# XiSHEN0220/RANSAC-Flow

Hardware: AMD Instinct MI355X
Metric: aligned image-pairs/sec @480×640, 1/2/4/8 MI355X; max-abs flow Δ vs ref (higher is better)
Workload: dtype f32

## Files before the change

### ransac-flow_amd/csrc/conv1x1s.hip

```cpp
#include "common.h"
#include "conv_epilogue.h"
#include "conv_split.h"
#include "conv_tile.h"
#include "group.h"

namespace {

struct C1SArgs {
    const float* in; const u32x4* wS; const float* scale; const float* shift; const float* res; float* out;
    int Cin, HW, Cout, act, Mpad;
    long long P;
    int tilesM, tilesP;
    int stride, Win, Wo, HWin;
};

template <int TM, int WM>
__device__ __forceinline__ void conv1x1_split_body(const C1SArgs& a, const unsigned bx, const unsigned) {
    constexpr int BM = 32 * TM * WM, BN = 128, KB = 16, NT = 128 * WM;
    constexpr bool WIDE = WM == 4;
    __shared__ u32x4 As[2][3][2][BM];
    __shared__ u32x4 Bs[2][3][2][BN];
    __shared__ float s_scale[BM], s_shift[BM];

    const int t = threadIdx.x, lane = t & 63, wave = t >> 6;
    const int wm = wave >> 1, wn = wave & 1;
    const int lrow = lane >> 5, lcol = lane & 31;
    const size_t HW = (size_t)a.HW, HWin = (size_t)a.HWin;
    const int nk = a.Cin / KB;

    const int bid = xcd_remap(bx, a.tilesM * a.tilesP);
    const int m0 = (bid % a.tilesM) * BM;
    const long long n0 = (long long)(bid / a.tilesM) * BN;
    SplitWeights<BM, NT> wa;
    wa.init(a.wS, a.Mpad, m0, WIDE);
    constexpr int NB = 2048 / NT;
    const int bh = t >> 7, bp = t & 127;
    const float* bsrc;
    {
        long long p = n0 + bp;
        if (p >= a.P) p = a.P - 1;
        const long long n = p / a.HW;
        int off = (int)(p - n * a.HW);
        if (a.stride != 1) { const int y = off / a.Wo, x = off - y * a.Wo; off = y * a.stride * a.Win + x * a.stride; }
        bsrc = a.in + ((size_t)n * a.Cin + NB * bh) * HWin + (size_t)off;
    }
    float rb[NB];
    auto load_stage = [&](int kb) {
        wa.load(kb, a.Mpad);
#pragma unroll
        for (int i = 0; i < NB; ++i) rb[i] = bsrc[(size_t)(kb * KB + i) * HWin];
    };
    auto store_stage = [&](int buf) {
        wa.store(&As[buf][0][0][0]);
        if constexpr (NB == 8) {
            u32x4 hi, mid, lo;
            split_word(rb, hi, mid, lo);
            Bs[buf][0][bh][bp] = hi;
            Bs[buf][1][bh][bp] = mid;
            Bs[buf][2][bh][bp] = lo;
        } else {
            u32x2 hi, mid, lo;
            split_word(rb, hi, mid, lo);
            u32x2* w = reinterpret_cast<u32x2*>(&Bs[buf][0][bh >> 1][bp]) + (bh & 1);
            w[0] = hi;
            w[4 * BN] = mid;
            w[8 * BN] = lo;
        }
    };
    stage_bn<BM>(s_scale, s_shift, a.scale, a.shift, m0, a.Cout);
    load_stage(0);
    store_stage(0);
    if (nk > 1) load_stage(1);
    __syncthreads();

    f32x16 acc[TM][2], low[TM][2];
    acc_zero(acc);
    acc_zero(low);

    for (int s = 0; s < nk; ++s) {
        const int cur = s & 1;
        bf16x8 af[3][TM], bf[3][2];
#pragma unroll
        for (int pc = 0; pc < 3; ++pc) {
#pragma unroll
            for (int i = 0; i < TM; ++i) af[pc][i] = as_frag(As[cur][pc][lrow][wm * TM * 32 + i * 32 + lcol]);
#pragma unroll
            for (int j = 0; j < 2; ++j) bf[pc][j] = as_frag(Bs[cur][pc][lrow][wn * 64 + j * 32 + lcol]);
        }
        if (s + 1 < nk) store_stage(cur ^ 1);
        if (s + 2 < nk) load_stage(s + 2);
        __builtin_amdgcn_sched_barrier(0);
#pragma unroll
        for (int i = 0; i < TM; ++i)
#pragma unroll
            for (int j = 0; j < 2; ++j) {
                low[i][j] = __builtin_amdgcn_mfma_f32_32x32x16_bf16(af[2][i], bf[0][j], low[i][j], 0, 0, 0);
                low[i][j] = __builtin_amdgcn_mfma_f32_32x32x16_bf16(af[0][i], bf[2][j], low[i][j], 0, 0, 0);
                low[i][j] = __builtin_amdgcn_mfma_f32_32x32x16_bf16(af[1][i], bf[1][j], low[i][j], 0, 0, 0);
            }
#pragma unroll
        for (int i = 0; i < TM; ++i)
#pragma unroll
            for (int j = 0; j < 2; ++j) {
                low[i][j] = __builtin_amdgcn_mfma_f32_32x32x16_bf16(af[1][i], bf[0][j], low[i][j], 0, 0, 0);
                low[i][j] = __builtin_amdgcn_mfma_f32_32x32x16_bf16(af[0][i], bf[1][j], low[i][j], 0, 0, 0);
                acc[i][j] = __builtin_amdgcn_mfma_f32_32x32x16_bf16(af[0][i], bf[0][j], acc[i][j], 0, 0, 0);
            }
        __builtin_amdgcn_sched_barrier(0);
        __syncthreads();
    }
    acc_add(acc, low);

    size_t pix_off[2];
    bool pix_ok[2];
    pix_linear<2>(pix_off, pix_ok, n0 + wn * 64 + lcol, a.P, a.HW, a.Cout);
    conv_epilogue<TM, 2, false>(acc, s_scale, s_shift, a.res, a.out, a.act, a.Cout, HW, m0, wm, lrow, pix_off, pix_ok, m0 + BM <= a.Cout);
}

template <int TM> using Split1 = RfxFamily<C1SArgs, conv1x1_split_body<TM, 2>, 256, 2>;
using Split1Wide = RfxFamily<C1SArgs, conv1x1_split_body<2, 4>, 512, 1>;

template <int TM>
__global__ __launch_bounds__((Split1<TM>::BLOCK), (Split1<TM>::min_waves())) void conv1x1_split_kernel(C1SArgs a) {
    conv1x1_split_body<TM, 2>(a, blockIdx.x, gridDim.x);
}

__global__ __launch_bounds__(Split1Wide::BLOCK, Split1Wide::min_waves()) void conv1x1_split_wide_kernel(C1SArgs a) {
    conv1x1_split_body<2, 4>(a, blockIdx.x, gridDim.x);
}

int c1s_tile_channels(long long P, int Cin, int Cout) {
    static const int mode = [] { const char* e = getenv("RFX_C1S_WIDE"); return e ? (atoi(e) == 0 ? 0 : 1) : -1; }();
    static const long long cus = [] {
        int dev = 0, n = 256;
        if (hipGetDevice(&dev) == hipSuccess) hipDeviceGetAttribute(&n, hipDeviceAttributeMultiprocessorCount, dev);
        return (long long)(n > 0 ? n : 256);
    }();
    if (Cout <= 64) return 64;
    if (Cout < 256 || mode == 0) return 128;
    if (mode == 1) return 256;
    if (Cin < 512) return 128;
    const long long tp = (P + 127) / 128, w = (Cout + 255) / 256 * tp, n = (Cout + 127) / 128 * tp;
    const long long rest = n % (2 * cus);
    const long long cost_wide = (w + cus - 1) / cus * 81, cost_128 = n / (2 * cus) * 100 + (rest == 0 ? 0 : rest <= cus ? 58 : 100);
    return cost_wide < cost_128 ? 256 : 128;
}

template <int TM, int WM>
int launch_split(C1SArgs& a, hipStream_t st) {
    constexpr int BM = 32 * TM * WM;
    a.tilesM = (a.Cout + BM - 1) / BM;
    a.tilesP = (int)((a.P + 127) / 128);
    const long long nwg = (long long)a.tilesM * a.tilesP;
    if (nwg > 0x7fffffffLL) return RFX_E_LIMIT;
    if constexpr (WM == 4) return Split1Wide::launch(conv1x1_split_wide_kernel, a, (unsigned)nwg, st);
    else return Split1<TM>::launch(conv1x1_split_kernel<TM>, a, (unsigned)nwg, st);
}

}

static int conv1x1_split_launch(const float* in, const void* wS, const float* scale, const float* shift, const float* residual,
                                float* out, int N, int Cin, int Hin, int Win, int Cout, int stride, int act, void* stream) {
    if (const int rc = conv_check_common(in, wS, out, N, Cin, Hin, Win, Cout, act)) return rc;
    if (stride != 1 && stride != 2) return RFX_E_ARG;
    const int Ho = (Hin - 1) / stride + 1, Wo = (Win - 1) / stride + 1;
    C1SArgs a;
    a.in = in; a.wS = reinterpret_cast<const u32x4*>(wS); a.scale = scale; a.shift = shift; a.res = residual; a.out = out;
    a.Cin = Cin; a.HW = Ho * Wo; a.Cout = Cout; a.act = act; a.Mpad = (Cout + 127) / 128 * 128;
    a.P = (long long)N * a.HW;
    a.stride = stride; a.Win = Win; a.Wo = Wo; a.HWin = Hin * Win;
    switch (c1s_tile_channels(a.P, Cin, Cout)) {
        case 256: return launch_split<2, 4>(a, rfx_stream(stream));
        case 128: return launch_split<2, 2>(a, rfx_stream(stream));
        default: return launch_split<1, 2>(a, rfx_stream(stream));
    }
}

extern "C" int rfx_conv1x1_split_tile_channels(int N, int Cin, int HWout, int Cout) {
    if (N <= 0 || Cin <= 0 || HWout <= 0 || Cout <= 0) return RFX_E_ARG;
    return c1s_tile_channels((long long)N * HWout, Cin, Cout);
}

extern "C" int rfx_conv1x1_split_f32(const float* in, const void* wS, const float* scale, const float* shift, const float* residual,
                                     float* out, int N, int Cin, int HW, int Cout, int act, void* stream) {
    return conv1x1_split_launch(in, wS, scale, shift, residual, out, N, Cin, 1, HW, Cout, 1, act, stream);
}

extern "C" int rfx_conv1x1_split_strided_f32(const float* in, const void* wS, const float* scale, const float* shift, const float* residual,
                                             float* out, int N, int Cin, int Hin, int Win, int Cout, int stride, int act, void* stream) {
    return conv1x1_split_launch(in, wS, scale, shift, residual, out, N, Cin, Hin, Win, Cout, stride, act, stream);
}
```

### ransac-flow_amd/csrc/conv_epilogue.h

```cpp
#pragma once
#include "common.h"

template <int TM, int TN>
__device__ __forceinline__ void conv_residual_prefetch(float (&pre)[TM * TN][16], const float* __restrict__ resp, size_t HWo,
                                                       int m0, int wm, int lrow, const size_t (&pix_off)[TN]) {
#pragma unroll
    for (int s = 0; s < TM * TN; ++s) {
        const size_t base = pix_off[s % TN] + (size_t)(m0 + (wm * TM + s / TN) * 32 + 4 * lrow) * HWo;
#pragma unroll
        for (int r = 0; r < 16; ++r) pre[s][r] = resp[base + (size_t)((r & 3) + 8 * (r >> 2)) * HWo];
    }
}

template <int TM, int TN, bool LEAN = false, bool PRE = false>
__device__ __forceinline__ void conv_epilogue(const f32x16 (&acc)[TM][TN], const float* s_scale, const float* s_shift,
                                              const float* __restrict__ resp, float* __restrict__ outp, int act,
                                              int Cout, size_t HWo, int m0, int wm, int lrow,
                                              const size_t (&pix_off)[TN], const bool (&pix_ok)[TN], bool m_full,
                                              const float (*pre)[16] = nullptr) {
    const bool has_res = resp != nullptr;
    if (m_full && act != RFX_ACT_SIGMOID) {
        const bool relu = act == RFX_ACT_RELU;
        constexpr int NS = TM * TN;
        auto sub_base = [&](int s) { return pix_off[s % TN] + (size_t)(m0 + (wm * TM + s / TN) * 32 + 4 * lrow) * HWo; };
        float rv[2][16];
        if (has_res && !LEAN && !PRE) {
            const size_t b0 = sub_base(0);
#pragma unroll
            for (int r = 0; r < 16; ++r) rv[0][r] = resp[b0 + (size_t)((r & 3) + 8 * (r >> 2)) * HWo];
        }
        float sc[16], sh[16];
#pragma unroll
        for (int s = 0; s < NS; ++s) {
            const int i = s / TN, j = s % TN;
            if (j == 0 || LEAN) {
                const int ml0 = (wm * TM + i) * 32 + 4 * lrow;
#pragma unroll
                for (int r = 0; r < 16; ++r) {
                    sc[r] = s_scale[ml0 + (r & 3) + 8 * (r >> 2)];
                    sh[r] = s_shift[ml0 + (r & 3) + 8 * (r >> 2)];
                }
            }
            if (has_res && LEAN && !PRE) {
                const size_t bc = sub_base(s);
#pragma unroll
                for (int r = 0; r < 16; ++r) rv[s & 1][r] = resp[bc + (size_t)((r & 3) + 8 * (r >> 2)) * HWo];
            }
            if (has_res && !LEAN && !PRE && s + 1 < NS) {
                const size_t bn = sub_base(s + 1);
#pragma unroll
                for (int r = 0; r < 16; ++r) rv[(s + 1) & 1][r] = resp[bn + (size_t)((r & 3) + 8 * (r >> 2)) * HWo];
            }
            const size_t base = sub_base(s);
            float v[16];
#pragma unroll
            for (int r = 0; r < 16; ++r) v[r] = fmaf(acc[i][j][r], sc[r], sh[r]);
            if (has_res) {
#pragma unroll
                for (int r = 0; r < 16; ++r) v[r] += PRE ? pre[s][r] : rv[s & 1][r];
            }
            if (relu) {
#pragma unroll
                for (int r = 0; r < 16; ++r) v[r] = v[r] > 0.0f ? v[r] : 0.0f;
            }
            if (pix_ok[j]) {
#pragma unroll
                for (int r = 0; r < 16; ++r) outp[base + (size_t)((r & 3) + 8 * (r >> 2)) * HWo] = v[r];
            }
            __builtin_amdgcn_sched_barrier(0);
        }
        return;
    }
#pragma unroll
    for (int j = 0; j < TN; ++j) {
#pragma unroll
        for (int i = 0; i < TM; ++i) {
            float rv[16];
#pragma unroll
            for (int r = 0; r < 16; ++r) {
                const int ml = (wm * TM + i) * 32 + (r & 3) + 8 * (r >> 2) + 4 * lrow;
                const int mc = (m0 + ml < Cout) ? (m0 + ml) : (Cout - 1);
                rv[r] = has_res ? resp[pix_off[j] + (size_t)mc * HWo] : 0.0f;
            }
#pragma unroll
            for (int r = 0; r < 16; ++r) {
                const int ml = (wm * TM + i) * 32 + (r & 3) + 8 * (r >> 2) + 4 * lrow;
                const int m = m0 + ml;
                float v = fmaf(acc[i][j][r], s_scale[ml], s_shift[ml]);
                if (has_res) v += rv[r];
                if (act == RFX_ACT_RELU) v = v > 0.0f ? v : 0.0f;
                else if (act == RFX_ACT_SIGMOID) v = 1.0f / (1.0f + expf(-v));
                if (pix_ok[j] && m < Cout) outp[pix_off[j] + (size_t)m * HWo] = v;
            }
        }
    }
}
```

### ransac-flow_amd/csrc/conv_tile.h

```cpp
#pragma once
#include "common.h"

template <int BM>
static __device__ __forceinline__ void stage_bn(float* s_scale, float* s_shift, const float* scale, const float* shift, int m0, int Cout) {
    const int t = threadIdx.x;
    if (t < BM) {
        const int m = m0 + t;
        s_scale[t] = (scale && m < Cout) ? scale[m] : 1.0f;
        s_shift[t] = (shift && m < Cout) ? shift[m] : 0.0f;
    }
}

template <int TM, int TN>
static __device__ __forceinline__ void acc_zero(f32x16 (&acc)[TM][TN]) {
#pragma unroll
    for (int i = 0; i < TM; ++i)
#pragma unroll
        for (int j = 0; j < TN; ++j)
#pragma unroll
            for (int r = 0; r < 16; ++r) acc[i][j][r] = 0.0f;
}
template <int TM, int TN>
static __device__ __forceinline__ void acc_add(f32x16 (&acc)[TM][TN], const f32x16 (&low)[TM][TN]) {
#pragma unroll
    for (int i = 0; i < TM; ++i)
#pragma unroll
        for (int j = 0; j < TN; ++j)
#pragma unroll
            for (int r = 0; r < 16; ++r) acc[i][j][r] += low[i][j][r];
}
template <int TM, int TN>
static __device__ __forceinline__ void acc_close_chunk(f32x16 (&tot)[TM][TN], f32x16 (&acc)[TM][TN]) {
#pragma unroll
    for (int i = 0; i < TM; ++i)
#pragma unroll
        for (int j = 0; j < TN; ++j)
#pragma unroll
            for (int r = 0; r < 16; ++r) { tot[i][j][r] += acc[i][j][r]; acc[i][j][r] = 0.0f; }
}

template <int TN>
static __device__ __forceinline__ void pix_linear(size_t (&pix_off)[TN], bool (&pix_ok)[TN], long long p0, long long P, int HW, int Cout) {
#pragma unroll
    for (int j = 0; j < TN; ++j) {
        long long pp = p0 + j * 32;
        pix_ok[j] = pp < P;
        if (!pix_ok[j]) pp = P - 1;
        const long long n = pp / HW;
        pix_off[j] = (size_t)n * Cout * (size_t)HW + (size_t)(pp - n * HW);
    }
}
```

Baseline: 165.6.

## Switch 1x1 split conv to 16x16x32 MFMA with triple-buffered two-step K loop

Replaces the 32x32x16 bf16 MFMA tiles with 16x16x32 ones, reorganising fragments so each iteration consumes two K blocks (one per lane group) from a triple-buffered shared-memory ring. Odd K counts are padded with a zero stage. Global loads and LDS stores are interleaved inside the row loop to overlap with MFMA work, and a new epilogue handles the 4-element accumulator layout. The aim is better MFMA throughput and latency hiding, at the cost of more shared memory (3 buffers) and more accumulator registers, which may reduce occupancy.

```diff
diff --git a/ransac-flow_amd/csrc/conv1x1s.hip b/ransac-flow_amd/csrc/conv1x1s.hip
--- a/ransac-flow_amd/csrc/conv1x1s.hip
+++ b/ransac-flow_amd/csrc/conv1x1s.hip
@@ -16,17 +16,17 @@
 
 template <int TM, int WM>
 __device__ __forceinline__ void conv1x1_split_body(const C1SArgs& a, const unsigned bx, const unsigned) {
-    constexpr int BM = 32 * TM * WM, BN = 128, KB = 16, NT = 128 * WM;
+    constexpr int BM = 32 * TM * WM, BN = 128, KB = 16, NT = 128 * WM, MI = 2 * TM, NJ = 4;
     constexpr bool WIDE = WM == 4;
-    __shared__ u32x4 As[2][3][2][BM];
-    __shared__ u32x4 Bs[2][3][2][BN];
+        __shared__ u32x4 As[3][3][2][BM];
+    __shared__ u32x4 Bs[3][3][2][BN];
     __shared__ float s_scale[BM], s_shift[BM];
 
     const int t = threadIdx.x, lane = t & 63, wave = t >> 6;
     const int wm = wave >> 1, wn = wave & 1;
-    const int lrow = lane >> 5, lcol = lane & 31;
+    const int g = lane >> 4, r16 = lane & 15;
     const size_t HW = (size_t)a.HW, HWin = (size_t)a.HWin;
-    const int nk = a.Cin / KB;
+    const int nk = a.Cin / KB, nkp = (nk + 1) & ~1;
 
     const int bid = xcd_remap(bx, a.tilesM * a.tilesP);
     const int m0 = (bid % a.tilesM) * BM;
@@ -46,9 +46,15 @@
     }
     float rb[NB];
     auto load_stage = [&](int kb) {
-        wa.load(kb, a.Mpad);
-#pragma unroll
-        for (int i = 0; i < NB; ++i) rb[i] = bsrc[(size_t)(kb * KB + i) * HWin];
+        if (kb < nk) {
+            wa.load(kb, a.Mpad);
+#pragma unroll
+            for (int i = 0; i < NB; ++i) rb[i] = bsrc[(size_t)(kb * KB + i) * HWin];
+        } else {
+            wa.load(nk - 1, a.Mpad);
+#pragma unroll
+            for (int i = 0; i < NB; ++i) rb[i] = 0.0f;
+        }
     };
     auto store_stage = [&](int buf) {
         wa.store(&As[buf][0][0][0]);
@@ -70,51 +76,71 @@
     stage_bn<BM>(s_scale, s_shift, a.scale, a.shift, m0, a.Cout);
     load_stage(0);
     store_stage(0);
-    if (nk > 1) load_stage(1);
+    load_stage(1);
+    store_stage(1);
+    if (2 < nkp) load_stage(2);
     __syncthreads();
 
-    f32x16 acc[TM][2], low[TM][2];
+    f32x4 acc[MI][NJ], low[MI][NJ];
     acc_zero(acc);
     acc_zero(low);
 
-    for (int s = 0; s < nk; ++s) {
-        const int cur = s & 1;
-        bf16x8 af[3][TM], bf[3][2];
+    int sa = 0, sb = 1, sc = 2;
+    for (int h0 = 0; h0 < nkp; h0 += 2) {
+        const int slot = g >> 1 ? sb : sa;
+        const u32x4* ap = &As[slot][0][g & 1][wm * TM * 32 + r16];
+        const u32x4* bq = &Bs[slot][0][g & 1][wn * 64 + r16];
+        bf16x8 af[MI][3], bf[3][NJ];
 #pragma unroll
         for (int pc = 0; pc < 3; ++pc) {
 #pragma unroll
-            for (int i = 0; i < TM; ++i) af[pc][i] = as_frag(As[cur][pc][lrow][wm * TM * 32 + i * 32 + lcol]);
-#pragma unroll
-            for (int j = 0; j < 2; ++j) bf[pc][j] = as_frag(Bs[cur][pc][lrow][wn * 64 + j * 32 + lcol]);
-        }
-        if (s + 1 < nk) store_stage(cur ^ 1);
-        if (s + 2 < nk) load_stage(s + 2);
-        __builtin_amdgcn_sched_barrier(0);
-#pragma unroll
-        for (int i = 0; i < TM; ++i)
-#pragma unroll
-            for (int j = 0; j < 2; ++j) {
-                low[i][j] = __builtin_amdgcn_mfma_f32_32x32x16_bf16(af[2][i], bf[0][j], low[i][j], 0, 0, 0);
-                low[i][j] = __builtin_amdgcn_mfma_f32_32x32x16_bf16(af[0][i], bf[2][j], low[i][j], 0, 0, 0);
-                low[i][j] = __builtin_amdgcn_mfma_f32_32x32x16_bf16(af[1][i], bf[1][j], low[i][j], 0, 0, 0);
-            }
-#pragma unroll
-        for (int i = 0; i < TM; ++i)
-#pragma unroll
-            for (int j = 0; j < 2; ++j) {
-                low[i][j] = __builtin_amdgcn_mfma_f32_32x32x16_bf16(af[1][i], bf[0][j], low[i][j], 0, 0, 0);
-                low[i][j] = __builtin_amdgcn_mfma_f32_32x32x16_bf16(af[0][i], bf[1][j], low[i][j], 0, 0, 0);
-                acc[i][j] = __builtin_amdgcn_mfma_f32_32x32x16_bf16(af[0][i], bf[0][j], acc[i][j], 0, 0, 0);
-            }
-        __builtin_amdgcn_sched_barrier(0);
+            for (int j = 0; j < NJ; ++j) bf[pc][j] = as_frag(bq[pc * 2 * BN + 16 * j]);
+            af[0][pc] = as_frag(ap[pc * 2 * BM]);
+        }
+#pragma unroll
+        for (int i = 0; i < MI; ++i) {
+            if (i == MI / 2 - 1) {
+                if (h0 + 2 < nkp) store_stage(sc);
+                if (h0 + 3 < nkp) load_stage(h0 + 3);
+            }
+            if (i == MI - 1) {
+                __syncthreads();
+                if (h0 + 3 < nkp) store_stage(sa);
+                if (h0 + 4 < nkp) load_stage(h0 + 4);
+            }
+            if (i + 1 < MI) {
+#pragma unroll
+                for (int pc = 0; pc < 3; ++pc) af[i + 1][pc] = as_frag(ap[pc * 2 * BM + 16 * (i + 1)]);
+            }
+            __builtin_amdgcn_sched_barrier(0);
+#pragma unroll
+            for (int j = 0; j < NJ; ++j) {
+                low[i][j] = __builtin_amdgcn_mfma_f32_16x16x32_bf16(af[i][2], bf[0][j], low[i][j], 0, 0, 0);
+                low[i][j] = __builtin_amdgcn_mfma_f32_16x16x32_bf16(af[i][0], bf[2][j], low[i][j], 0, 0, 0);
+                low[i][j] = __builtin_amdgcn_mfma_f32_16x16x32_bf16(af[i][1], bf[1][j], low[i][j], 0, 0, 0);
+            }
+#pragma unroll
+            for (int j = 0; j < NJ; ++j) {
+                low[i][j] = __builtin_amdgcn_mfma_f32_16x16x32_bf16(af[i][1], bf[0][j], low[i][j], 0, 0, 0);
+                low[i][j] = __builtin_amdgcn_mfma_f32_16x16x32_bf16(af[i][0], bf[1][j], low[i][j], 0, 0, 0);
+                acc[i][j] = __builtin_amdgcn_mfma_f32_16x16x32_bf16(af[i][0], bf[0][j], acc[i][j], 0, 0, 0);
+            }
+            __builtin_amdgcn_sched_barrier(0);
+        }
         __syncthreads();
+        const int s0 = sa;
+        sa = sc; sc = sb; sb = s0;
     }
     acc_add(acc, low);
 
-    size_t pix_off[2];
-    bool pix_ok[2];
-    pix_linear<2>(pix_off, pix_ok, n0 + wn * 64 + lcol, a.P, a.HW, a.Cout);
-    conv_epilogue<TM, 2, false>(acc, s_scale, s_shift, a.res, a.out, a.act, a.Cout, HW, m0, wm, lrow, pix_off, pix_ok, m0 + BM <= a.Cout);
+    int te = threadIdx.x;
+    asm volatile("" : "+v"(te));
+    const int e_wm = te >> 7, e_wn = (te >> 6) & 1, e_g = (te >> 4) & 3, e_r16 = te & 15;
+    size_t pix_off[NJ];
+    bool pix_ok[NJ];
+    pix_linear<NJ, 16>(pix_off, pix_ok, n0 + e_wn * 64 + e_r16, a.P, a.HW, a.Cout);
+    conv_epilogue16<MI, NJ>(acc, s_scale, s_shift, a.res, a.out, a.act, a.Cout, HW, m0, e_wm * TM * 32, e_g, pix_off, pix_ok,
+                            m0 + BM <= a.Cout);
 }
 
 template <int TM> using Split1 = RfxFamily<C1SArgs, conv1x1_split_body<TM, 2>, 256, 2>;
diff --git a/ransac-flow_amd/csrc/conv_epilogue.h b/ransac-flow_amd/csrc/conv_epilogue.h
--- a/ransac-flow_amd/csrc/conv_epilogue.h
+++ b/ransac-flow_amd/csrc/conv_epilogue.h
@@ -95,3 +95,68 @@
         }
     }
 }
+
+template <int TM, int TN>
+__device__ __forceinline__ void conv_epilogue16(const f32x4 (&acc)[TM][TN], const float* s_scale, const float* s_shift,
+                                                const float* __restrict__ resp, float* __restrict__ outp, int act,
+                                                int Cout, size_t HWo, int m0, int mw0, int g,
+                                                const size_t (&pix_off)[TN], const bool (&pix_ok)[TN], bool m_full) {
+    const bool has_res = resp != nullptr;
+    if (m_full && act != RFX_ACT_SIGMOID) {
+        const bool relu = act == RFX_ACT_RELU;
+        auto row_base = [&](int i) { return (size_t)(m0 + mw0 + 16 * i + 4 * g) * HWo; };
+        float rv[2][TN][4];
+        auto fetch = [&](int i) {
+            const size_t b = row_base(i);
+#pragma unroll
+            for (int j = 0; j < TN; ++j)
+#pragma unroll
+                for (int r = 0; r < 4; ++r) rv[i & 1][j][r] = resp[b + pix_off[j] + (size_t)r * HWo];
+        };
+        if (has_res) fetch(0);
+#pragma unroll
+        for (int i = 0; i < TM; ++i) {
+            float sc[4], sh[4];
+#pragma unroll
+            for (int r = 0; r < 4; ++r) {
+                sc[r] = s_scale[mw0 + 16 * i + 4 * g + r];
+                sh[r] = s_shift[mw0 + 16 * i + 4 * g + r];
+            }
+            if (has_res && i + 1 < TM) fetch(i + 1);
+            const size_t b = row_base(i);
+#pragma unroll
+            for (int j = 0; j < TN; ++j) {
+                float v[4];
+#pragma unroll
+                for (int r = 0; r < 4; ++r) {
+                    v[r] = fmaf(acc[i][j][r], sc[r], sh[r]);
+                    if (has_res) v[r] += rv[i & 1][j][r];
+                    if (relu) v[r] = v[r] > 0.0f ? v[r] : 0.0f;
+                }
+                if (pix_ok[j]) {
+#pragma unroll
+                    for (int r = 0; r < 4; ++r) outp[b + pix_off[j] + (size_t)r * HWo] = v[r];
+                }
+            }
+            __builtin_amdgcn_sched_barrier(0);
+        }
+        return;
+    }
+#pragma unroll
+    for (int i = 0; i < TM; ++i) {
+#pragma unroll
+        for (int j = 0; j < TN; ++j) {
+#pragma unroll
+            for (int r = 0; r < 4; ++r) {
+                const int ml = mw0 + 16 * i + 4 * g + r;
+                const int m = m0 + ml;
+                const int mc = m < Cout ? m : Cout - 1;
+                float v = fmaf(acc[i][j][r], s_scale[ml], s_shift[ml]);
+                if (has_res) v += resp[pix_off[j] + (size_t)mc * HWo];
+                if (act == RFX_ACT_RELU) v = v > 0.0f ? v : 0.0f;
+                else if (act == RFX_ACT_SIGMOID) v = 1.0f / (1.0f + expf(-v));
+                if (pix_ok[j] && m < Cout) outp[pix_off[j] + (size_t)m * HWo] = v;
+            }
+        }
+    }
+}
diff --git a/ransac-flow_amd/csrc/conv_tile.h b/ransac-flow_amd/csrc/conv_tile.h
--- a/ransac-flow_amd/csrc/conv_tile.h
+++ b/ransac-flow_amd/csrc/conv_tile.h
@@ -11,23 +11,23 @@
     }
 }
 
-template <int TM, int TN>
-static __device__ __forceinline__ void acc_zero(f32x16 (&acc)[TM][TN]) {
+template <typename V, int TM, int TN>
+static __device__ __forceinline__ void acc_zero(V (&acc)[TM][TN]) {
 #pragma unroll
     for (int i = 0; i < TM; ++i)
 #pragma unroll
         for (int j = 0; j < TN; ++j)
 #pragma unroll
-            for (int r = 0; r < 16; ++r) acc[i][j][r] = 0.0f;
+            for (int r = 0; r < (int)(sizeof(V) / 4); ++r) acc[i][j][r] = 0.0f;
 }
-template <int TM, int TN>
-static __device__ __forceinline__ void acc_add(f32x16 (&acc)[TM][TN], const f32x16 (&low)[TM][TN]) {
+template <typename V, int TM, int TN>
+static __device__ __forceinline__ void acc_add(V (&acc)[TM][TN], const V (&low)[TM][TN]) {
 #pragma unroll
     for (int i = 0; i < TM; ++i)
 #pragma unroll
         for (int j = 0; j < TN; ++j)
 #pragma unroll
-            for (int r = 0; r < 16; ++r) acc[i][j][r] += low[i][j][r];
+            for (int r = 0; r < (int)(sizeof(V) / 4); ++r) acc[i][j][r] += low[i][j][r];
 }
 template <int TM, int TN>
 static __device__ __forceinline__ void acc_close_chunk(f32x16 (&tot)[TM][TN], f32x16 (&acc)[TM][TN]) {
@@ -39,11 +39,11 @@
             for (int r = 0; r < 16; ++r) { tot[i][j][r] += acc[i][j][r]; acc[i][j][r] = 0.0f; }
 }
 
-template <int TN>
+template <int TN, int STEP = 32>
 static __device__ __forceinline__ void pix_linear(size_t (&pix_off)[TN], bool (&pix_ok)[TN], long long p0, long long P, int HW, int Cout) {
 #pragma unroll
     for (int j = 0; j < TN; ++j) {
-        long long pp = p0 + j * 32;
+        long long pp = p0 + j * STEP;
         pix_ok[j] = pp < P;
         if (!pix_ok[j]) pp = P - 1;
         const long long n = pp / HW;
```

Result: no change. 167.2, median of 6 (+0.9%).
